# TGAC/KAT

Hardware: AMD Instinct MI355X
Metric: k-mers/sec (whole node) for kat comp reads-vs-assembly k=27 (higher is better)
Workload: dtype u64

## Files before the change

kat_amd/csrc/kg_count.hip:

```cpp
#include "kg_host.hpp"
#include "kg_ingest.hpp"
#include "kg_kernels.hpp"
#include "kg_partition.hpp"
#include "kg_partition_wide.hpp"

#include <condition_variable>
#include <deque>
#include <mutex>
#include <thread>


static const uint64_t g_test_sweep_thr = hook("KATGPU_TEST_SWEEP_THR") ? strtoull(hook("KATGPU_TEST_SWEEP_THR"), nullptr, 10) : 0;
static const uint64_t g_test_max_starts = hook("KATGPU_TEST_MAX_STARTS") ? strtoull(hook("KATGPU_TEST_MAX_STARTS"), nullptr, 10) : 0;

namespace kg {
static __global__ void __launch_bounds__(256)
k_sweep(DevTable t, uint32_t thr, unsigned long long* scratch) {
    uint32_t mx = 0;
    const uint64_t stride = (uint64_t)gridDim.x * blockDim.x;
    for (uint64_t i = (uint64_t)blockIdx.x * blockDim.x + threadIdx.x; i < t.cap; i += stride) {
        uint32_t c = t.counts[i];
        if (c >= thr) {
            uint64_t key = t.keys[i];
            uint32_t take = (c / thr) * thr;
// ... 51 lines not shown
    if ((reinterpret_cast<uintptr_t>(dev_bases) & 15) == 0)
        hipLaunchKernelGGL(k_count<true>, dim3(grid), dim3(COUNT_BLOCK), 0, c->stream, t->dev(), dev_bases, (uint64_t)n, n_chunks);
    else
        hipLaunchKernelGGL(k_count<false>, dim3(grid), dim3(COUNT_BLOCK), 0, c->stream, t->dev(), dev_bases, (uint64_t)n, n_chunks);
    HIPCHK(c, hipGetLastError());
    return KATGPU_OK;
}



static const uint64_t g_part_min_starts = getenv("KATGPU_PART_MIN_STARTS") ? strtoull(getenv("KATGPU_PART_MIN_STARTS"), nullptr, 10) : (32ULL << 20);
static const uint64_t g_test_round_items = hook("KATGPU_TEST_ROUND_ITEMS") ? strtoull(hook("KATGPU_TEST_ROUND_ITEMS"), nullptr, 10) : 0;
static const double g_arena_fraction = getenv("KATGPU_ARENA_FRACTION") ? std::min(0.95, std::max(0.05, atof(getenv("KATGPU_ARENA_FRACTION")))) : 0.85;
static const uint32_t g_p1_wgs = hook("KATGPU_P1_WGS") ? std::max<uint32_t>(1, (uint32_t)strtoul(hook("KATGPU_P1_WGS"), nullptr, 10)) : 3;
static const uint32_t g_l1_fast = hook("KATGPU_L1_FAST") ? (uint32_t)strtoul(hook("KATGPU_L1_FAST"), nullptr, 10) : 1;
static const uint32_t g_test_l1_cpb = hook("KATGPU_TEST_L1_CPB") ? (uint32_t)strtoul(hook("KATGPU_TEST_L1_CPB"), nullptr, 10) : 0;
static const uint32_t g_p2_fast = hook("KATGPU_P2_FAST") ? (uint32_t)strtoul(hook("KATGPU_P2_FAST"), nullptr, 10) : 1;
static const uint64_t g_test_p2_ovf_cap = hook("KATGPU_TEST_P2_OVF_CAP") ? strtoull(hook("KATGPU_TEST_P2_OVF_CAP"), nullptr, 10) : 0;
static const uint32_t g_test_spill_mod = hook("KATGPU_TEST_SPILL_MOD") ? (uint32_t)strtoul(hook("KATGPU_TEST_SPILL_MOD"), nullptr, 10) : 0;
static const uint64_t g_test_ap_seg = hook_u64("KATGPU_TEST_AP_SEG", 0) & ~3ULL;
static const uint32_t g_apply_per_cu = (uint32_t)hook_u64("KATGPU_APPLY_PER_CU", 0);
static const uint64_t g_fresh_max_pct = hook_u64("KATGPU_FRESH_MAX_PCT", 100);
static const bool g_l1b_stamp = hook_u64("KATGPU_L1B_STAMP", 0) != 0;
static const bool g_p2x_stamp = hook_u64("KATGPU_P2X_STAMP", 0) != 0;
static const bool g_p2_stamp = hook_u64("KATGPU_P2_STAMP", 0) != 0;
static const bool g_apply_stamp = hook_u64("KATGPU_APPLY_STAMP", 0) != 0;

static bool part_geometry(const DevTable& d, PartGeom* g) {
    g->R = d.n_regions; g->S = d.region_slots; g->P1 = d.p1; g->P2 = d.p2; g->l2 = d.l2;
    g->b_lo = 0; g->b_hi = d.p1;
// ... 219 lines not shown
    switch (g.hb) {
    case 0: rc = apply_kv12_shape<0>(a, blk, big, fresh, hooked); break;
    case 1: rc = apply_kv12_shape<1>(a, blk, big, fresh, hooked); break;
    case 2: rc = apply_kv12_shape<2>(a, blk, big, fresh, hooked); break;
    case 4: rc = apply_kv12_shape<4>(a, blk, big, fresh, hooked); break;
    }
    if (rc) return rc;
    HIPCHK(c, hipGetLastError());
    return KATGPU_OK;
}

constexpr uint8_t GUARD_BYTE = 0xA5;
struct PartArena {
    uint32_t hb, passes, n_cu; uint64_t regions; bool blocks_shape; double per_item_max; size_t small_bytes;
    uint32_t* hist1; uint64_t* offs; uint64_t* l1_off; uint64_t* off2; uint32_t* cnt2; uint64_t* bend; unsigned long long* spill_n; unsigned long long* ovf_n;
    uint8_t* l1_buf;
    uint8_t* l2_buf;
    uint64_t* ovf_buf; uint64_t ovf_cap;
    ArenaCarve cv;
    size_t round_items, l1_bytes, l2_items;
    PartArena(const PartGeom& g0, uint32_t k, uint32_t W, uint32_t n_cu_) : hb(g0.hb), passes(std::max<uint32_t>(1, g0.P1 / pass_buckets(g0.P1, n_cu_))), n_cu(n_cu_), regions(g0.R), blocks_shape(l1_blocks_shape(g0, k)) {
        per_item_max = arena_bytes_per_item(hb, passes, false, false);
        small_bytes = align_up((size_t)W * MAX_PARTS * 4, 256) + align_up((size_t)W * MAX_PARTS * 8, 256) +
                      align_up((MAX_PARTS + 1) * 8, 256) + align_up(((size_t)MAX_PARTS * MAX_PARTS + 1) * 8, 256) +
                      align_up((size_t)MAX_PARTS * MAX_PARTS * 4, 256) + align_up((size_t)MAX_PARTS * 8, 256) + align_up((size_t)MAX_PARTS * 4, 256) + 256;
    }
    size_t fixed_bytes(uint32_t W) const { return small_bytes + (size_t)arena_fixed_bytes(hb, passes, W, n_cu, false, false); }
    bool carve_from(uint8_t* a, size_t arena_bytes, uint32_t W, size_t want_items) {
        uint8_t* const a0 = a;
        hist1 = carve<uint32_t>(a, (size_t)W * MAX_PARTS * 4);
        offs = carve<uint64_t>(a, (size_t)W * MAX_PARTS * 8);
        l1_off = carve<uint64_t>(a, (MAX_PARTS + 1) * 8);
        off2 = carve<uint64_t>(a, ((size_t)MAX_PARTS * MAX_PARTS + 1) * 8);
        cnt2 = carve<uint32_t>(a, (size_t)MAX_PARTS * MAX_PARTS * 4);
        bend = carve<uint64_t>(a, (size_t)MAX_PARTS * 8);
        carve<uint32_t>(a, (size_t)MAX_PARTS * 4);
        spill_n = carve<unsigned long long>(a, STAMP_AREA * 8);
        ovf_n = spill_n + 1;
        if ((size_t)(a - a0) > small_bytes || arena_bytes <= small_bytes) return false;
        cv = arena_carve(arena_bytes - small_bytes, want_items, hb, passes, W, n_cu, regions, blocks_shape, g_l1_fast, g_test_p2_ovf_cap);
        round_items = cv.round_items; l1_bytes = cv.l1_bytes; l2_items = cv.l2_items; ovf_cap = cv.ovf_cap;
        l1_buf = a;
        l2_buf = l1_buf + cv.l1_bytes + ARENA_GUARD;
        ovf_buf = (uint64_t*)(l2_buf + cv.l2_bytes + ARENA_GUARD);
        return (size_t)((uint8_t*)(ovf_buf + ovf_cap) + ARENA_GUARD - a0) <= arena_bytes;
    }
    uint8_t* guard(int i) const { return i == 0 ? l1_buf + cv.l1_bytes : i == 1 ? l2_buf + cv.l2_bytes : (uint8_t*)(ovf_buf + ovf_cap); }
};
static const char* const GUARD_NAME[3] = {"level-1 buffer", "level-2 buffer", "overflow list"};
static int guards_set(katgpu_ctx* c, const PartArena& A) {
    if (!g_testing) return KATGPU_OK;
    for (int i = 0; i < 3; ++i) HIPCHK(c, hipMemsetAsync(A.guard(i), GUARD_BYTE, ARENA_GUARD, c->stream));
    return KATGPU_OK;
// ... 23 lines not shown
    return t->dv.k == 32 && !t->dv.canonical ? restore_ones(t) : KATGPU_OK;
}

enum class L1Edition { Blocks, SegLean512, SegLean1024, SegPlain512, SegPlain1024, ExactLean, ExactPlain };
static const char* const L1_EDITION_NAME[] = {"Blocks", "SegLean512", "SegLean1024", "SegPlain512", "SegPlain1024", "ExactLean", "ExactPlain"};
struct L1Plan {
    L1Edition edition; bool seg ; uint32_t wgs ; uint64_t n_tiles, tiles_per_wg;
    uint64_t seg_cap, cap_plain, stride64;
};
static L1Plan plan_level1(const PartGeom& g, uint32_t k, size_t m, uint64_t est_items, uint32_t W, uint32_t n_cu, size_t l1_bytes, bool seg_wanted) {
    const bool lean = g_l1_lean && lean_applies(k, g.pl.n1);
    const bool pb512 = g.P1 <= 512;
    const bool l1b = l1_blocks_shape(g, k);
    const uint64_t n_tiles = (m + P1_TILE_STARTS - 1) / P1_TILE_STARTS;
    L1Plan pl;
    pl.wgs = l1b ? n_cu : W;
    pl.n_tiles = l1b ? (m + L1B_TILE_STARTS - 1) / L1B_TILE_STARTS : n_tiles;
    const L1Segments sg = l1_segments(l1b, g.P1, g.hb1, pl.wgs, est_items, (pl.n_tiles + pl.wgs - 1) / pl.wgs, g_test_l1_cpb, l1_bytes);
    pl.cap_plain = sg.cap_plain; pl.seg_cap = sg.seg_cap; pl.stride64 = sg.stride;
    pl.seg = seg_wanted && sg.fits;
    if (pl.seg) pl.edition = l1b ? L1Edition::Blocks : lean ? (pb512 ? L1Edition::SegLean512 : L1Edition::SegLean1024) : (pb512 ? L1Edition::SegPlain512 : L1Edition::SegPlain1024);
    else { pl.edition = lean ? L1Edition::ExactLean : L1Edition::ExactPlain; pl.wgs = W; pl.n_tiles = n_tiles; }
    pl.tiles_per_wg = (pl.n_tiles + pl.wgs - 1) / pl.wgs;
    return pl;
}
static int launch_l1_scatter(katgpu_table* t, const PartGeom& g, const L1Plan& l1, const PartArena& A, const uint8_t* p, uint64_t nb) {
    katgpu_ctx* c = t->ctx;
    auto blocks = [&](auto kern, unsigned long long* stamps) {
        return launch_lds(c, kern, dim3(l1.wgs), dim3(L1B_THREADS), sizeof(P1BLds), sizeof(P1BLds), t->dv, g, p, nb, l1.n_tiles, l1.tiles_per_wg,
                          A.l1_buf, (uint32_t)(l1.seg_cap / L1B_ITEMS), (uint32_t)l1.stride64, A.ovf_buf, A.ovf_n, A.ovf_cap, stamps);
    };
    auto segmented = [&](auto kern) {
        hipLaunchKernelGGL(kern, dim3(l1.wgs), dim3(P1_BLOCK), 0, c->stream, t->dv, g, p, nb, l1.n_tiles, l1.tiles_per_wg, (const uint64_t*)nullptr, (const uint64_t*)nullptr, A.l1_buf,
                           (uint32_t)l1.seg_cap, (uint32_t)l1.stride64, (uint32_t)l1.cap_plain, A.ovf_buf, A.ovf_n, A.ovf_cap);
        return KATGPU_OK;
    };
    auto exact = [&](auto kern) {
        hipLaunchKernelGGL(kern, dim3(l1.wgs), dim3(P1_BLOCK), 0, c->stream, t->dv, g, p, nb, l1.n_tiles, l1.tiles_per_wg, (const uint64_t*)A.offs, (const uint64_t*)A.l1_off, A.l1_buf,
                           0u, 0u, 0u, (uint64_t*)nullptr, (unsigned long long*)nullptr, (uint64_t)0);
        return KATGPU_OK;
    };
    switch (l1.edition) {
    case L1Edition::Blocks:
        if (!g_l1b_stamp) return blocks(k_p1b_scatter<false>, nullptr);
        return with_stamps(c, A.spill_n + STAMP_AT, 10, &STAMPS_L1B, [&](unsigned long long* st) { return blocks(k_p1b_scatter<true>, st); });
    case L1Edition::SegLean512:   return segmented(k_p1v2_scatter<true, true, 512>);
    case L1Edition::SegLean1024:  return segmented(k_p1v2_scatter<true, true, MAX_PARTS>);
    case L1Edition::SegPlain512:  return segmented(k_p1v2_scatter<true, false, 512>);
    case L1Edition::SegPlain1024: return segmented(k_p1v2_scatter<true, false, MAX_PARTS>);
    case L1Edition::ExactLean:    return exact(k_p1v2_scatter<false, true, MAX_PARTS>);
    case L1Edition::ExactPlain:   return exact(k_p1v2_scatter<false, false, MAX_PARTS>);
    }
    return KATGPU_OK;
}
static int level1(katgpu_table* t, const PartGeom& g, const L1Plan& l1, const PartArena& A, size_t cap_items, const uint8_t* p, size_t m, double items_per_start, uint64_t* items) {
    katgpu_ctx* c = t->ctx;
    const uint64_t nb = m + t->dv.k - 1;
    if (l1.seg) {
        int rc;
        if (l1.stride64 * g.P1 > A.l1_bytes || (uint64_t)l1.wgs * (l1.edition == L1Edition::Blocks ? l1.seg_cap / L1B_ITEMS * L1B_BYTES : (4 + g.hb1) * l1.seg_cap) > l1.stride64)
// ... 11 lines not shown
    HIPCHK(c, hipMemcpyAsync(items, &A.l1_off[g.P1], sizeof *items, hipMemcpyDeviceToHost, c->stream));
    HIPCHK(c, hipStreamSynchronize(c->stream));
    if (g_trace) fprintf(stderr, "[katgpu] partition round: %zu starts -> %llu items (buffer %zu items, arena %.1f GB, ratio %.3f; capacity %zu items, %s, stride 0)\n", m, (unsigned long long)*items, A.round_items, c->arena_bytes / 1e9, items_per_start,
                         cap_items, L1_EDITION_NAME[(int)l1.edition]);
    if (*items > cap_items) return t->dv.k == 32 && !t->dv.canonical ? restore_ones(t) : KATGPU_OK;
    if (!*items) return KATGPU_OK;
    if (l1_bucket_base(*items, g.P1) + 32 > A.l1_bytes)
        return fail(c, KATGPU_ERR_DEVICE, "partition round: %llu items of an exact level 1 end beyond the level-1 buffer of %zu bytes", (unsigned long long)*items, A.l1_bytes);
    ScopedTimer tm(c, KATGPU_K_PART_L1S, *items);
    return launch_l1_scatter(t, g, l1, A, p, nb);
}

enum class L1Items { Groups , WideGroups , Blocks  };
static const char* const L1_ITEMS_NAME[] = {"Groups", "WideGroups", "Blocks"};
enum L2Family : uint32_t { L2_BLOCKS = 1 , L2_ONE_PASS = 2 , L2_EXACT = 4  };
struct L2Pass { katgpu_ctx* c; const PartGeom& g; const PartArena& A; uint32_t grid; L1Items src; uint64_t seg_slots; uint32_t* families ; };
template <typename K>
static int p2_one_pass(const L2Pass& x, K kern, size_t lds, unsigned long long* stamps = nullptr) {
    return launch_lds(x.c, kern, dim3(x.grid), dim3(PART_BLOCK), lds, lds, x.g, x.A.l1_off, x.A.l1_buf, x.A.l2_buf, x.A.off2, x.A.cnt2, x.A.ovf_buf, x.A.ovf_n, x.A.ovf_cap, x.seg_slots, stamps);
}
template <typename K>
static int p2_exact(const L2Pass& x, K kern, size_t lds) {
    return launch_lds(x.c, kern, dim3(x.grid), dim3(PART_BLOCK), lds, lds, x.g, x.A.l1_off, x.A.l1_buf, x.A.l2_buf, x.A.off2, x.seg_slots, x.A.bend);
}
template <int HB>
static int launch_l2_hb(const L2Pass& x, bool one_pass) {
    constexpr size_t lds_e = sizeof(P2Lds<HB>), lds_f = sizeof(typename P2FastLds<HB>::type);
    unsigned long long* const stamps = x.A.spill_n + STAMP_AT;
    if (x.families) *x.families |= !one_pass ? L2_EXACT : x.src == L1Items::Blocks && HB == 1 ? L2_BLOCKS : L2_ONE_PASS;
    switch (x.src) {
    case L1Items::Blocks:
        if constexpr (HB == 4) break;
        else if (!one_pass) return p2_exact(x, k_p2<HB, false, true>, lds_e);
        else if constexpr (HB != 1) return p2_one_pass(x, k_p2_fast<HB, false, false, true>, lds_f);
        else if (!g_p2x_stamp) return p2_one_pass(x, k_p2x_fast<false>, sizeof(P2XLds));
        else return with_stamps(x.c, stamps, 10, &STAMPS_P2X, [&](unsigned long long* st) { return p2_one_pass(x, k_p2x_fast<true>, sizeof(P2XLds), st); });
    case L1Items::WideGroups: return one_pass ? p2_one_pass(x, k_p2_fast<HB, true>, lds_f) : p2_exact(x, k_p2<HB, true>, lds_e);
    case L1Items::Groups:
        if constexpr (HB == 1) if (one_pass && g_p2_stamp) return with_stamps(x.c, stamps, 6, &STAMPS_P2, [&](unsigned long long* st) { return p2_one_pass(x, k_p2_fast<1, false, true>, lds_f, st); });
        return one_pass ? p2_one_pass(x, k_p2_fast<HB, false>, lds_f) : p2_exact(x, k_p2<HB, false>, lds_e);
    }
    return fail(x.c, KATGPU_ERR_DEVICE, "level 2 from blocked level-1 items: item width %u", x.g.hb);
}
static int launch_l2(const L2Pass& x, bool one_pass) {
    switch (x.g.hb) {
    case 0: return launch_l2_hb<0>(x, one_pass);
    case 1: return launch_l2_hb<1>(x, one_pass);
    case 2: return launch_l2_hb<2>(x, one_pass);
    case 4: return launch_l2_hb<4>(x, one_pass);
    }
    return fail(x.c, KATGPU_ERR_DEVICE, "level 2: item width %u", x.g.hb);
// ... 39 lines not shown
    };
    uint32_t step = pass_buckets(g.P1, (uint32_t)c->n_cu);
    auto fits = [&](uint32_t st) { for (uint32_t b = 0; b < g.P1; b += st) if (pass_extent(b, std::min(g.P1, b + st)) > A.l2_items) return false; return true; };
    if (!seg && A.cv.big) {
        g.l2_trim = 0;
        if (!fits(step) && l2_trims(g.hb, items, g.R)) g.l2_trim = 1;
    }
    while (step > 1 && !fits(step)) step = (step + 1) / 2;
    if (!fits(step)) {
        *end = RoundEnd::DirectPath;
        return seg || (t->dv.k == 32 && !t->dv.canonical) ? restore_ones(t) : KATGPU_OK;
    }
    const bool try_fast0 = *p2_fast_ok && (g_p2_fast == 2 || items / g.R >= 1024);
    unsigned long long ovf_total = ovf_l1;
    uint32_t l2_families = 0;
    ApplyForm ap{};
    if (g_trace && g.P1 > step) fprintf(stderr, "[katgpu]   level 2 + apply in %u passes of %u buckets (level-2 buffer: %zu items)\n", (g.P1 + step - 1) / step, step, A.l2_items);
    for (uint32_t b_lo = 0; b_lo < g.P1; b_lo += step) {
        g.b_lo = b_lo; g.b_hi = std::min(g.P1, b_lo + step);
        const uint64_t pass_items = std::max<uint64_t>(1, (uint64_t)((double)items * (g.b_hi - g.b_lo) / g.P1));
        auto l1_at = [&](uint32_t b) -> uint64_t { return seg ? (uint64_t)b * g.l1_stride : l1_bucket_base(lbeg(b), b); };
        uint64_t* spill_buf = (uint64_t*)(A.l1_buf + l1_at(b_lo));
        g.spill_cap = (l1_at(g.b_hi) - l1_at(b_lo)) / 8;
        const bool try_fast = try_fast0 && *p2_fast_ok;
        const L2Pass x{c, g, A, std::min<uint32_t>(g.b_hi - g.b_lo, (uint32_t)c->n_cu), src, seg_slots, &l2_families};
        HIPCHK(c, hipMemsetAsync(A.spill_n, 0, sizeof(unsigned long long), c->stream));
        int rc = KATGPU_OK;
        if (try_fast) { ScopedTimer tm(c, KATGPU_K_PART_L2, pass_items); rc = launch_l2(x, true); }
        if (rc) return rc;
        L2Next next = L2Next::Exact;
        unsigned long long overflowed = ovf_total;
        if (try_fast || (seg && b_lo == 0)) {
            rc = read_overflow(t, A, seg, try_fast, ovf_l1, &ovf_total, &overflowed, &next);
            if (rc) return rc;
            if (next == L2Next::RedoRound) { *end = RoundEnd::RedoExactL1; return KATGPU_OK; }
            if (next == L2Next::FallBackExact) *p2_fast_ok = false;
        }
        const bool runs = next == L2Next::UseCnt2;
        if (!runs) { ScopedTimer tm(c, KATGPU_K_PART_L2, pass_items); rc = launch_l2(x, false); }
        if (rc) return rc;
        ovf_total = overflowed;
        {
            ScopedTimer tm(c, KATGPU_K_PART_APPLY, pass_items);
            rc = launch_apply(t, g, A.off2, A.l2_buf, spill_buf, A.spill_n, runs ? A.cnt2 : nullptr, runs ? nullptr : A.bend, items, &ap);
// ... 527 lines not shown
```

kat_amd/csrc/kg_l1_blocks.hpp:

```cpp
#pragma once

namespace kg {

constexpr uint32_t L1B_ITEMS = 10, L1B_BYTES = 64;
constexpr int L1B_THREADS = 1024;
constexpr int L1B_TILE_BYTES = L1B_THREADS * PART_ITEMS;
constexpr int L1B_TILE_STARTS = L1B_TILE_BYTES - CHUNK_OVERLAP;
constexpr int L1B_LANES_WITH_STARTS = L1B_TILE_STARTS / PART_ITEMS;
constexpr uint32_t L1B_PB = 512;
constexpr uint32_t L1B_POOL = 1712;

struct P1BLds {
    uint32_t hist[L1B_PB + 64];
    uint2 gb[L1B_PB + 64];
    uint32_t where[L1B_POOL];
    uint32_t wave_tot[L1B_THREADS / 64];
    uint32_t code[L1B_THREADS + 2];
    uint16_t bad[L1B_THREADS + 2];
    __attribute__((aligned(16))) uint32_t img[(L1B_PB + L1B_POOL) * 16];
};
static_assert(sizeof(P1BLds) <= 160 * 1024 - 1280, "one workgroup per CU");

__device__ __forceinline__ uint32_t l1b_lo_at(uint32_t B, uint32_t s) { return B + 3 * (s >> 1) + (s & 1); }
__device__ __forceinline__ uint32_t l1b_hi_at(uint32_t B, uint32_t s) { return 2 * (B + 3 * (s >> 1) + 2) + (s & 1); }
// ... 8 lines not shown
#pragma unroll
    for (uint32_t i = 0; i < 4; ++i) {
        const uint32_t b = (tid_o & ~63u) + 16 * i + ((tid_o & 63) >> 2);
        const uint2 d = L.gb[b];
        if (d.x & 0xFFFFu) {
            const u32x4 a = *reinterpret_cast<const u32x4*>(&L.img[b * 16 + (tid_o & 3) * 4]);
            *reinterpret_cast<u32x4*>(&L.img[d.y * 16 + (tid_o & 3) * 4]) = a;
        }
    }
}

template <bool STAMP = false >
__global__ void __launch_bounds__(L1B_THREADS)
k_p1b_scatter(DevTable t, PartGeom g, const uint8_t* __restrict__ bases, uint64_t n, uint64_t n_tiles, uint64_t tiles_per_wg,
              uint8_t* __restrict__ l1_buf, uint32_t segb , uint32_t bucket_stride ,
              uint64_t* __restrict__ ovf_buf, unsigned long long* __restrict__ ovf_n, uint64_t ovf_cap, unsigned long long* __restrict__ stamps) {
    constexpr uint32_t PB = L1B_PB;
    unsigned long long st[10] = {0, 0, 0, 0, 0, 0, 0, 0, 0, 0}, tq = 0;
    auto stamp = [&](int i) { if (STAMP) { const unsigned long long x = (unsigned long long)clock64(); st[i] += x - tq; tq = x; } };
    extern __shared__ __attribute__((aligned(16))) unsigned char lds_raw[];
    P1BLds& L = *reinterpret_cast<P1BLds*>(lds_raw);
    const uint32_t tid = threadIdx.x, P = g.P1, k = t.k;
    uint16_t* const img16 = reinterpret_cast<uint16_t*>(L.img);
    uint8_t* const seg0 = l1_buf + (uint64_t)blockIdx.x * segb * L1B_BYTES;
    const LeanGeom lg = lean_geom(k, t.canonical != 0, g.pl.n1);
    auto overflow = [&](uint32_t b, uint32_t lo, uint32_t hi) {
        const unsigned long long at = atomicAdd(ovf_n, 1ULL);
        if (at < ovf_cap) ovf_buf[at] = place_key_r1(b, ((uint64_t)hi << 32) | lo, g.pl);
    };
    if (tid < PB + 64) { L.hist[tid] = 0; L.gb[tid] = uint2{0u, 0u}; }
    if (tid < PB) L.img[tid * 16 + 15] = 0;
// ... 148 lines not shown
        const bool room = cur < segb;
        if (cn && !room) {
            for (uint32_t s = 0; s < cn; ++s) overflow(tid, L.img[l1b_lo_at(tid * 16, s)], img16[l1b_hi_at(tid * 16, s)]);
        }
        if (cn && room) for (uint32_t s = cn; s < L1B_ITEMS; ++s) { L.img[l1b_lo_at(tid * 16, s)] = 0xFFFFFFFFu; img16[l1b_hi_at(tid * 16, s)] = 0xFFFFu; }
        L.gb[tid].x = cn && room ? 1u : 0u;
    }
    lds_barrier();
    for (uint32_t qi = tid; qi < 4 * P; qi += L1B_THREADS) {
        const uint32_t b = qi >> 2, w = qi & 3;
        const uint32_t cur = L.img[b * 16 + 15];
        u32x4 v = *reinterpret_cast<const u32x4*>(&L.img[b * 16 + 4 * w]);
        if (w == 3) v.w = 0xFFFFFFFFu;
        if (L.gb[b].x) *reinterpret_cast<u32x4*>(seg0 + ((uint64_t)b * bucket_stride + ((uint64_t)cur << 6) + 16 * w)) = v;
    }
    lds_barrier();
    {
        const uint32_t wave = tid >> 6, lane = tid & 63;
        for (uint32_t b = wave; b < P; b += L1B_THREADS / 64) {
            const uint32_t from = L.img[b * 16 + 15] + L.gb[b].x;
            uint8_t* seg = seg0 + (uint64_t)b * bucket_stride;
            for (uint32_t q = from * 4 + lane; q < segb * 4; q += 64) *reinterpret_cast<u32x4*>(seg + (uint64_t)q * 16) = u32x4{0xFFFFFFFFu, 0xFFFFFFFFu, 0xFFFFFFFFu, 0xFFFFFFFFu};
        }
    }
}

}
```

kat_amd/csrc/kg_l2_blocks.hpp:

```cpp
#pragma once

namespace kg {

constexpr int L2X_N = 14;
constexpr uint32_t L2X_TILE = L2X_N * PART_BLOCK;
constexpr uint32_t L2X_POOL = 1252;

struct P2XLds {
    uint32_t hist[MAX_PARTS + 64];
    uint2 gb[MAX_PARTS];
    uint32_t where[L2X_POOL];
    uint32_t wave_tot[32];
    __attribute__((aligned(64))) uint32_t img[(MAX_PARTS + L2X_POOL) * 16];
};
static_assert(sizeof(P2XLds) <= 160 * 1024 - 256 && offsetof(P2XLds, img) % 64 == 0, "LDS");
static_assert(PART_BLOCK == MAX_PARTS, "thread b is sub-bucket b");

template <bool STAMP = false >
__global__ void __launch_bounds__(PART_BLOCK)
k_p2x_fast(PartGeom g, const uint64_t* __restrict__ l1_off, const uint8_t* __restrict__ l1_buf, uint8_t* __restrict__ l2_buf,
           uint64_t* __restrict__ off2, uint32_t* __restrict__ cnt2, uint64_t* __restrict__ ovf_buf, unsigned long long* __restrict__ ovf_n,
           uint64_t ovf_cap, uint64_t seg_slots, unsigned long long* __restrict__ stamps) {
    constexpr int N = L2X_N;
    constexpr uint32_t PB = MAX_PARTS, TILE_CAP = L2Fmt<1>::TILE ;
    extern __shared__ __attribute__((aligned(64))) unsigned char lds_raw[];
    P2XLds& L = *reinterpret_cast<P2XLds*>(lds_raw);
    unsigned char* const img8 = reinterpret_cast<unsigned char*>(L.img);
    const uint32_t tid = threadIdx.x, P = g.P2;
    unsigned long long st[10] = {0, 0, 0, 0, 0, 0, 0, 0, 0, 0}, tq = 0;
    auto stamp = [&](int i) { if (STAMP) { const unsigned long long x = (unsigned long long)clock64(); st[i] += x - tq; tq = x; } };
    uint64_t beg0, n0, nr0;
    l1_bucket_range(g, l1_off, seg_slots, g.b_lo, beg0, n0, nr0);
    uint32_t tid_o = tid;
    for (uint32_t b1 = g.b_lo + blockIdx.x; b1 < g.b_hi; b1 += gridDim.x) {
        uint64_t beg, n_items, n_real;
        const uint8_t* bucket = l1_buf + l1_bucket_range(g, l1_off, seg_slots, b1, beg, n_items, n_real);
        const uint64_t cap = p2_region_cap(n_real, P, TILE_CAP, L2_BLOCK_ITEMS, g.l2_trim != 0);
        const uint64_t obase = p2_out_base(beg, b1, P, TILE_CAP, L2_BLOCK_ITEMS, g.l2_trim != 0) - p2_out_base(beg0, g.b_lo, P, TILE_CAP, L2_BLOCK_ITEMS, g.l2_trim != 0);
        uint8_t* const runs = l2_buf + l2_lo_at<1>(obase >> 2);
        const uint32_t capb = (uint32_t)(cap / L2_BLOCK_ITEMS);
        lds_barrier();
        asm volatile("" : "+v"(tid_o));
        L.hist[tid_o] = 0; L.gb[tid_o] = uint2{0u, 0u};
        if (tid < 64) L.hist[PB + tid_o] = 0;
        L.img[tid_o * 16 + 15] = 0;
        if (tid < P) off2[(uint64_t)b1 * P + tid_o] = obase + (uint64_t)tid * cap;
        uint32_t n_out = 0;
        constexpr int OUT_STEPS = (L2X_POOL + PART_BLOCK / 4 - 1) / (PART_BLOCK / 4);
        static_assert(OUT_STEPS <= N / 2, "a step per pair of the ranking's items");
        struct OutStep { u32x4 v; uint32_t where; };
        auto out_read = [&](int it, OutStep& o) {
            asm volatile("" : "+v"(tid_o));
            const uint32_t s = min((tid_o >> 2) + (uint32_t)it * (PART_BLOCK / 4), L2X_POOL - 1);
            o.where = L.where[s];
            o.v = *reinterpret_cast<const u32x4*>(&L.img[(PB + s) * 16 + (tid_o & 3) * 4]);
        };
        auto out_store = [&](int it, const OutStep& o) {
            asm volatile("" : "+v"(tid_o));
            if ((tid_o >> 2) + (uint32_t)it * (PART_BLOCK / 4) < n_out)
                *reinterpret_cast<u32x4*>(runs + (((uint64_t)o.where << 6) | ((tid_o & 3) * 16))) = o.v;
        };
        RawTileB<N> raw;
        p2_tile_issue_l1b<N>(bucket, 0, raw);
        for (uint64_t tbeg = 0; tbeg < n_items; tbeg += L2X_TILE) {
            if (STAMP) tq = (unsigned long long)clock64();
            TileItems<N, false> key;
            const uint32_t valid = p2_tile_decode_l1b<N>(tbeg, n_items, raw, key);
            {
#pragma unroll
                for (int j = 0; j < N; ++j) asm volatile("" : "+v"(key.lo[j]));
#pragma unroll
                for (int j = 0; j < N / 2; ++j) asm volatile("" : "+v"(key.hi[j]));
            }
            p2_tile_issue_l1b<N>(bucket, tbeg + L2X_TILE, raw);
            stamp(0);
            lds_barrier();
            stamp(1);
            uint32_t br[N];
            {
                uint32_t rk[N];
                const uint32_t dump = PB + (tid & 63);
                OutStep o;
#pragma unroll
                for (int j = 0; j < N; ++j) {
                    if (j % 2 == 0 && j / 2 < OUT_STEPS) out_read(j / 2, o);
                    const uint32_t b = place_digit2_of(key.r1(j), g.pl) & (PB - 1);
                    rk[j] = atomicAdd(&L.hist[(valid >> j & 1) ? b : dump], 1u);
                    br[j] = b << 16;
                    if (j >= 2) br[j - 2] |= rk[j - 2];
// ... 114 lines not shown
```

kat_amd/csrc/kg_partition.hpp:

```cpp
#pragma once
#include "kg_kernels.hpp"
#include "kg_l1_lean.hpp"
#include "kg_apply_lean.hpp"
#include "kg_arena_plan.hpp"

#include <cstddef>
#include <type_traits>

namespace kg {

constexpr int PART_BLOCK = 1024;
constexpr int PART_ITEMS = BASES_PER_LANE;
constexpr int TILE_ITEMS = PART_BLOCK * PART_ITEMS;
constexpr int L1_TILE_BYTES = TILE_ITEMS;
constexpr int L1_TILE_STARTS = L1_TILE_BYTES - CHUNK_OVERLAP;
constexpr int L1_LANES_WITH_STARTS = L1_TILE_STARTS / PART_ITEMS;

__device__ __forceinline__ void lds_barrier() { asm volatile("s_waitcnt lgkmcnt(0)\n\ts_barrier" ::: "memory"); }
__device__ __forceinline__ void spill_put(uint64_t* __restrict__ spill, unsigned long long* __restrict__ spill_n, uint64_t cap, uint64_t key) {
    const unsigned long long at = atomicAdd(spill_n, 1ULL);
    if (at < cap) spill[at] = key;
}

struct PartGeom {
// ... 526 lines not shown
        for (int off = 32; off > 0; off >>= 1) ones += __shfl_down(ones, off, 64);
        if ((tid & 63) == 0 && ones) atomicAdd((unsigned long long*)&t.ctrs[CTR_ONES], (unsigned long long)ones);
    }
}

}
#include "kg_l1_blocks.hpp"
namespace kg {

__device__ __forceinline__ uint64_t l1_bucket_range(const PartGeom& g, const uint64_t* __restrict__ l1_off, uint64_t seg_slots, uint32_t b1, uint64_t& first, uint64_t& n_items, uint64_t& n_real) {
    if (seg_slots) { first = (uint64_t)b1 * g.l1_real; n_items = seg_slots; n_real = g.l1_real; return (uint64_t)b1 * g.l1_stride; }
    first = l1_off[b1]; n_items = n_real = l1_off[b1 + 1] - first;
    return l1_bucket_base(first, b1);
}

template <int N, bool W1>
struct TileItems {
    uint32_t lo[N];
    uint32_t hi[W1 ? N : N / 2];
    __device__ __forceinline__ uint64_t r1(int j) const {
        const uint32_t h = W1 ? hi[j] : (hi[j >> 1] >> (16 * (j & 1))) & 0xFFFFu;
        return ((uint64_t)h << 32) | lo[j];
    }
};
template <int N>
__device__ __forceinline__ uint32_t p2_tile_load_wide(const uint8_t* __restrict__ bucket, uint64_t tbeg, uint64_t n_items, TileItems<N, true>& it) {
    static_assert(N % 2 == 0, "pairs");
    const uint64_t left = n_items - tbeg;
    const uint32_t t_items = left < (uint64_t)N * PART_BLOCK ? (uint32_t)left : (uint32_t)N * PART_BLOCK;
    const uint8_t* mine = bucket + (tbeg + 2 * threadIdx.x) * 8;
// ... 55 lines not shown
    p2_tile_issue_narrow<N>(hb1, bucket, tbeg, r);
    return p2_tile_decode_narrow<N>(hb1, tbeg, n_items, r, it);
}
typedef uint32_t u32x3 __attribute__((ext_vector_type(3)));
typedef u32x3 u32x3_a4 __attribute__((aligned(4)));
template <int N> struct RawTileB { u32x3 v[N / 2]; };
template <int N>
__device__ __forceinline__ void p2_tile_issue_l1b(const uint8_t* __restrict__ bucket, uint64_t tbeg, RawTileB<N>& r) {
    const uint32_t p0 = (uint32_t)(tbeg >> 1) + threadIdx.x;
    uint32_t blk = __umulhi(p0, 0xCCCCCCCDu) >> 2, part = p0 - 5 * blk;
#pragma unroll
    for (int u = 0; u < N / 2; ++u) {
        r.v[u] = *reinterpret_cast<const u32x3_a4*>(bucket + (uint32_t)((blk << 6) + 12 * part));
        blk += PART_BLOCK / 5; part += PART_BLOCK % 5;
        if (part >= 5) { part -= 5; ++blk; }
    }
}
template <int N>
__device__ __forceinline__ uint32_t p2_tile_decode_l1b(uint64_t tbeg, uint64_t n_items, const RawTileB<N>& r, TileItems<N, false>& it) {
    const uint64_t left = tbeg < n_items ? n_items - tbeg : 0;
    const uint32_t t_items = left < (uint64_t)N * PART_BLOCK ? (uint32_t)left : (uint32_t)N * PART_BLOCK;
    uint32_t valid = 0;
#pragma unroll
    for (int u = 0; u < N / 2; ++u) {
        const uint32_t i0 = 2 * ((uint32_t)u * PART_BLOCK + threadIdx.x);
        it.lo[2 * u] = r.v[u].x; it.lo[2 * u + 1] = r.v[u].y; it.hi[u] = r.v[u].z;
        uint32_t ta = (i0 < t_items && !(r.v[u].x == 0xFFFFFFFFu && (r.v[u].z & 0xFFFFu) == 0xFFFFu)) ? 1u : 0u;
        uint32_t tb = (i0 + 1 < t_items && !(r.v[u].y == 0xFFFFFFFFu && (r.v[u].z >> 16) == 0xFFFFu)) ? 1u : 0u;
        asm volatile("" : "+v"(ta), "+v"(tb));
        valid |= (ta << (2 * u)) | (tb << (2 * u + 1));
// ... 1091 lines not shown
```

Measured before the change: 114.9 billion.

## Read only filled level-1 segments via per-bucket fill prefix sums

The level-1 blocks scatter no longer pads every unused segment tail with 0xFF sentinels. It records each workgroup's filled block count per bucket, and a small scan kernel turns these into per-bucket prefix sums. The one-pass level-2 reader for hb==1 uses the prefix sums to map logical blocks onto physical segment positions, so it only walks filled blocks. Other level-2 paths still get a lazy padding kernel. This removes padding writes and reads of empty capacity, at the cost of an extra scan launch and more address arithmetic in the L2 tile loads.

```diff
diff --git a/kat_amd/csrc/kg_count.hip b/kat_amd/csrc/kg_count.hip
--- a/kat_amd/csrc/kg_count.hip
+++ b/kat_amd/csrc/kg_count.hip
@@ -89,6 +89,7 @@
 static const double g_arena_fraction = getenv("KATGPU_ARENA_FRACTION") ? std::min(0.95, std::max(0.05, atof(getenv("KATGPU_ARENA_FRACTION")))) : 0.85;
 static const uint32_t g_p1_wgs = hook("KATGPU_P1_WGS") ? std::max<uint32_t>(1, (uint32_t)strtoul(hook("KATGPU_P1_WGS"), nullptr, 10)) : 3;
 static const uint32_t g_l1_fast = hook("KATGPU_L1_FAST") ? (uint32_t)strtoul(hook("KATGPU_L1_FAST"), nullptr, 10) : 1;
+static const uint32_t g_test_l1b_wgs = (uint32_t)hook_u64("KATGPU_TEST_L1B_WGS", 0);
 static const uint32_t g_test_l1_cpb = hook("KATGPU_TEST_L1_CPB") ? (uint32_t)strtoul(hook("KATGPU_TEST_L1_CPB"), nullptr, 10) : 0;
 static const uint32_t g_p2_fast = hook("KATGPU_P2_FAST") ? (uint32_t)strtoul(hook("KATGPU_P2_FAST"), nullptr, 10) : 1;
 static const uint64_t g_test_p2_ovf_cap = hook("KATGPU_TEST_P2_OVF_CAP") ? strtoull(hook("KATGPU_TEST_P2_OVF_CAP"), nullptr, 10) : 0;
@@ -338,6 +339,7 @@
 struct PartArena {
     uint32_t hb, passes, n_cu; uint64_t regions; bool blocks_shape; double per_item_max; size_t small_bytes;
     uint32_t* hist1; uint64_t* offs; uint64_t* l1_off; uint64_t* off2; uint32_t* cnt2; uint64_t* bend; unsigned long long* spill_n; unsigned long long* ovf_n;
+    uint32_t* l1_fill; uint32_t* l1_cum;
     uint8_t* l1_buf;
     uint8_t* l2_buf;
     uint64_t* ovf_buf; uint64_t ovf_cap;
@@ -347,8 +349,11 @@
         per_item_max = arena_bytes_per_item(hb, passes, false, false);
         small_bytes = align_up((size_t)W * MAX_PARTS * 4, 256) + align_up((size_t)W * MAX_PARTS * 8, 256) +
                       align_up((MAX_PARTS + 1) * 8, 256) + align_up(((size_t)MAX_PARTS * MAX_PARTS + 1) * 8, 256) +
-                      align_up((size_t)MAX_PARTS * MAX_PARTS * 4, 256) + align_up((size_t)MAX_PARTS * 8, 256) + align_up((size_t)MAX_PARTS * 4, 256) + 256;
-    }
+                      align_up((size_t)MAX_PARTS * MAX_PARTS * 4, 256) + align_up((size_t)MAX_PARTS * 8, 256) + align_up((size_t)MAX_PARTS * 4, 256) + 256 +
+                      align_up(fill_bytes(), 256) + align_up(cum_bytes(), 256);
+    }
+    size_t fill_bytes() const { return (size_t)n_cu * L1B_PB * 4; }
+    size_t cum_bytes() const { return ((size_t)n_cu + 1) * L1B_PB * 4; }
     size_t fixed_bytes(uint32_t W) const { return small_bytes + (size_t)arena_fixed_bytes(hb, passes, W, n_cu, false, false); }
     bool carve_from(uint8_t* a, size_t arena_bytes, uint32_t W, size_t want_items) {
         uint8_t* const a0 = a;
@@ -361,6 +366,8 @@
         carve<uint32_t>(a, (size_t)MAX_PARTS * 4);
         spill_n = carve<unsigned long long>(a, STAMP_AREA * 8);
         ovf_n = spill_n + 1;
+        l1_fill = carve<uint32_t>(a, fill_bytes());
+        l1_cum = carve<uint32_t>(a, cum_bytes());
         if ((size_t)(a - a0) > small_bytes || arena_bytes <= small_bytes) return false;
         cv = arena_carve(arena_bytes - small_bytes, want_items, hb, passes, W, n_cu, regions, blocks_shape, g_l1_fast, g_test_p2_ovf_cap);
         round_items = cv.round_items; l1_bytes = cv.l1_bytes; l2_items = cv.l2_items; ovf_cap = cv.ovf_cap;
@@ -414,7 +421,7 @@
     const bool l1b = l1_blocks_shape(g, k);
     const uint64_t n_tiles = (m + P1_TILE_STARTS - 1) / P1_TILE_STARTS;
     L1Plan pl;
-    pl.wgs = l1b ? n_cu : W;
+    pl.wgs = l1b ? (g_test_l1b_wgs ? std::min(g_test_l1b_wgs, n_cu) : n_cu) : W;
     pl.n_tiles = l1b ? (m + L1B_TILE_STARTS - 1) / L1B_TILE_STARTS : n_tiles;
     const L1Segments sg = l1_segments(l1b, g.P1, g.hb1, pl.wgs, est_items, (pl.n_tiles + pl.wgs - 1) / pl.wgs, g_test_l1_cpb, l1_bytes);
     pl.cap_plain = sg.cap_plain; pl.seg_cap = sg.seg_cap; pl.stride64 = sg.stride;
@@ -428,7 +435,7 @@
     katgpu_ctx* c = t->ctx;
     auto blocks = [&](auto kern, unsigned long long* stamps) {
         return launch_lds(c, kern, dim3(l1.wgs), dim3(L1B_THREADS), sizeof(P1BLds), sizeof(P1BLds), t->dv, g, p, nb, l1.n_tiles, l1.tiles_per_wg,
-                          A.l1_buf, (uint32_t)(l1.seg_cap / L1B_ITEMS), (uint32_t)l1.stride64, A.ovf_buf, A.ovf_n, A.ovf_cap, stamps);
+                          A.l1_buf, (uint32_t)(l1.seg_cap / L1B_ITEMS), (uint32_t)l1.stride64, A.ovf_buf, A.ovf_n, A.ovf_cap, A.l1_fill, stamps);
     };
     auto segmented = [&](auto kern) {
         hipLaunchKernelGGL(kern, dim3(l1.wgs), dim3(P1_BLOCK), 0, c->stream, t->dv, g, p, nb, l1.n_tiles, l1.tiles_per_wg, (const uint64_t*)nullptr, (const uint64_t*)nullptr, A.l1_buf,
@@ -441,9 +448,14 @@
         return KATGPU_OK;
     };
     switch (l1.edition) {
-    case L1Edition::Blocks:
-        if (!g_l1b_stamp) return blocks(k_p1b_scatter<false>, nullptr);
-        return with_stamps(c, A.spill_n + STAMP_AT, 10, &STAMPS_L1B, [&](unsigned long long* st) { return blocks(k_p1b_scatter<true>, st); });
+    case L1Edition::Blocks: {
+        if (g_testing) HIPCHK(c, hipMemsetAsync(A.l1_buf, 0x01, l1.stride64 * g.P1, c->stream));
+        int rc = !g_l1b_stamp ? blocks(k_p1b_scatter<false>, nullptr)
+                              : with_stamps(c, A.spill_n + STAMP_AT, 10, &STAMPS_L1B, [&](unsigned long long* st) { return blocks(k_p1b_scatter<true>, st); });
+        if (rc) return rc;
+        hipLaunchKernelGGL(k_l1_fill_scan, dim3(g.P1), dim3(64), 0, c->stream, (const uint32_t*)A.l1_fill, A.l1_cum, l1.wgs);
+        return KATGPU_OK;
+    }
     case L1Edition::SegLean512:   return segmented(k_p1v2_scatter<true, true, 512>);
     case L1Edition::SegLean1024:  return segmented(k_p1v2_scatter<true, true, MAX_PARTS>);
     case L1Edition::SegPlain512:  return segmented(k_p1v2_scatter<true, false, 512>);
@@ -485,10 +497,27 @@
 enum class L1Items { Groups , WideGroups , Blocks  };
 static const char* const L1_ITEMS_NAME[] = {"Groups", "WideGroups", "Blocks"};
 enum L2Family : uint32_t { L2_BLOCKS = 1 , L2_ONE_PASS = 2 , L2_EXACT = 4  };
-struct L2Pass { katgpu_ctx* c; const PartGeom& g; const PartArena& A; uint32_t grid; L1Items src; uint64_t seg_slots; uint32_t* families ; };
+struct L2Pass {
+    katgpu_ctx* c; const PartGeom& g; const PartArena& A; uint32_t grid; L1Items src; uint64_t seg_slots; uint32_t* families ;
+    uint32_t wgs, segb;
+    bool* padded;
+};
 template <typename K>
 static int p2_one_pass(const L2Pass& x, K kern, size_t lds, unsigned long long* stamps = nullptr) {
     return launch_lds(x.c, kern, dim3(x.grid), dim3(PART_BLOCK), lds, lds, x.g, x.A.l1_off, x.A.l1_buf, x.A.l2_buf, x.A.off2, x.A.cnt2, x.A.ovf_buf, x.A.ovf_n, x.A.ovf_cap, x.seg_slots, stamps);
+}
+template <typename K>
+static int p2_blocks(const L2Pass& x, K kern, unsigned long long* stamps = nullptr) {
+    const size_t lds = sizeof(P2XLds);
+    return launch_lds(x.c, kern, dim3(x.grid), dim3(PART_BLOCK), lds, lds, x.g, x.A.l1_off, x.A.l1_buf, x.A.l2_buf, x.A.off2, x.A.cnt2, x.A.ovf_buf, x.A.ovf_n, x.A.ovf_cap, x.seg_slots,
+                      (const uint32_t*)x.A.l1_cum, x.wgs, x.segb, stamps);
+}
+static int pad_blocks(const L2Pass& x) {
+    if (*x.padded) return KATGPU_OK;
+    hipLaunchKernelGGL(k_l1_pad_segments, dim3((x.g.P1 - x.g.b_lo) * x.wgs), dim3(256), 0, x.c->stream, (const uint32_t*)x.A.l1_fill, x.A.l1_buf, x.wgs, x.segb, x.g.l1_stride, x.g.b_lo);
+    *x.padded = true;
+    if (g_trace) fprintf(stderr, "[katgpu]   level-1 segments of buckets %u .. %u filled up with \"no item\" (k_l1_pad_segments): the reader takes whole segments\n", x.g.b_lo, x.g.P1 - 1);
+    return KATGPU_OK;
 }
 template <typename K>
 static int p2_exact(const L2Pass& x, K kern, size_t lds) {
@@ -502,10 +531,10 @@
     switch (x.src) {
     case L1Items::Blocks:
         if constexpr (HB == 4) break;
-        else if (!one_pass) return p2_exact(x, k_p2<HB, false, true>, lds_e);
-        else if constexpr (HB != 1) return p2_one_pass(x, k_p2_fast<HB, false, false, true>, lds_f);
-        else if (!g_p2x_stamp) return p2_one_pass(x, k_p2x_fast<false>, sizeof(P2XLds));
-        else return with_stamps(x.c, stamps, 10, &STAMPS_P2X, [&](unsigned long long* st) { return p2_one_pass(x, k_p2x_fast<true>, sizeof(P2XLds), st); });
+        else if (!one_pass) { int rc = pad_blocks(x); return rc ? rc : p2_exact(x, k_p2<HB, false, true>, lds_e); }
+        else if constexpr (HB != 1) { int rc = pad_blocks(x); return rc ? rc : p2_one_pass(x, k_p2_fast<HB, false, false, true>, lds_f); }
+        else if (!g_p2x_stamp) return p2_blocks(x, k_p2x_fast<false>);
+        else return with_stamps(x.c, stamps, 10, &STAMPS_P2X, [&](unsigned long long* st) { return p2_blocks(x, k_p2x_fast<true>, st); });
     case L1Items::WideGroups: return one_pass ? p2_one_pass(x, k_p2_fast<HB, true>, lds_f) : p2_exact(x, k_p2<HB, true>, lds_e);
     case L1Items::Groups:
         if constexpr (HB == 1) if (one_pass && g_p2_stamp) return with_stamps(x.c, stamps, 6, &STAMPS_P2, [&](unsigned long long* st) { return p2_one_pass(x, k_p2_fast<1, false, true>, lds_f, st); });
@@ -575,6 +604,14 @@
     const bool try_fast0 = *p2_fast_ok && (g_p2_fast == 2 || items / g.R >= 1024);
     unsigned long long ovf_total = ovf_l1;
     uint32_t l2_families = 0;
+    bool padded = false;
+    const uint32_t segb = src == L1Items::Blocks ? (uint32_t)(l1.seg_cap / L1B_ITEMS) : 0u;
+    std::vector<uint32_t> h_cum;
+    if (g_trace && src == L1Items::Blocks) {
+        h_cum.resize((size_t)g.P1 * (l1.wgs + 1));
+        HIPCHK(c, hipMemcpyAsync(h_cum.data(), A.l1_cum, h_cum.size() * 4, hipMemcpyDeviceToHost, c->stream));
+        HIPCHK(c, hipStreamSynchronize(c->stream));
+    }
     ApplyForm ap{};
     if (g_trace && g.P1 > step) fprintf(stderr, "[katgpu]   level 2 + apply in %u passes of %u buckets (level-2 buffer: %zu items)\n", (g.P1 + step - 1) / step, step, A.l2_items);
     for (uint32_t b_lo = 0; b_lo < g.P1; b_lo += step) {
@@ -584,11 +621,17 @@
         uint64_t* spill_buf = (uint64_t*)(A.l1_buf + l1_at(b_lo));
         g.spill_cap = (l1_at(g.b_hi) - l1_at(b_lo)) / 8;
         const bool try_fast = try_fast0 && *p2_fast_ok;
-        const L2Pass x{c, g, A, std::min<uint32_t>(g.b_hi - g.b_lo, (uint32_t)c->n_cu), src, seg_slots, &l2_families};
+        const L2Pass x{c, g, A, std::min<uint32_t>(g.b_hi - g.b_lo, (uint32_t)c->n_cu), src, seg_slots, &l2_families, l1.wgs, segb, &padded};
         HIPCHK(c, hipMemsetAsync(A.spill_n, 0, sizeof(unsigned long long), c->stream));
         int rc = KATGPU_OK;
         if (try_fast) { ScopedTimer tm(c, KATGPU_K_PART_L2, pass_items); rc = launch_l2(x, true); }
         if (rc) return rc;
+        if (try_fast && !h_cum.empty() && g.hb == 1) {
+            unsigned long long read = 0;
+            for (uint32_t b = g.b_lo; b < g.b_hi; ++b) read += h_cum[(size_t)b * (l1.wgs + 1) + l1.wgs];
+            fprintf(stderr, "[katgpu]   level 2 walked buckets %u .. %u compacted: %llu blocks read of %llu blocks of capacity (%u segments of %u per bucket)\n", g.b_lo, g.b_hi - 1, read,
+                    (unsigned long long)(g.b_hi - g.b_lo) * l1.wgs * segb, l1.wgs, segb);
+        }
         L2Next next = L2Next::Exact;
         unsigned long long overflowed = ovf_total;
         if (try_fast || (seg && b_lo == 0)) {
diff --git a/kat_amd/csrc/kg_l1_blocks.hpp b/kat_amd/csrc/kg_l1_blocks.hpp
--- a/kat_amd/csrc/kg_l1_blocks.hpp
+++ b/kat_amd/csrc/kg_l1_blocks.hpp
@@ -46,7 +46,8 @@
 __global__ void __launch_bounds__(L1B_THREADS)
 k_p1b_scatter(DevTable t, PartGeom g, const uint8_t* __restrict__ bases, uint64_t n, uint64_t n_tiles, uint64_t tiles_per_wg,
               uint8_t* __restrict__ l1_buf, uint32_t segb , uint32_t bucket_stride ,
-              uint64_t* __restrict__ ovf_buf, unsigned long long* __restrict__ ovf_n, uint64_t ovf_cap, unsigned long long* __restrict__ stamps) {
+              uint64_t* __restrict__ ovf_buf, unsigned long long* __restrict__ ovf_n, uint64_t ovf_cap, uint32_t* __restrict__ fill ,
+              unsigned long long* __restrict__ stamps) {
     constexpr uint32_t PB = L1B_PB;
     unsigned long long st[10] = {0, 0, 0, 0, 0, 0, 0, 0, 0, 0}, tq = 0;
     auto stamp = [&](int i) { if (STAMP) { const unsigned long long x = (unsigned long long)clock64(); st[i] += x - tq; tq = x; } };
@@ -225,15 +226,7 @@
         if (w == 3) v.w = 0xFFFFFFFFu;
         if (L.gb[b].x) *reinterpret_cast<u32x4*>(seg0 + ((uint64_t)b * bucket_stride + ((uint64_t)cur << 6) + 16 * w)) = v;
     }
-    lds_barrier();
-    {
-        const uint32_t wave = tid >> 6, lane = tid & 63;
-        for (uint32_t b = wave; b < P; b += L1B_THREADS / 64) {
-            const uint32_t from = L.img[b * 16 + 15] + L.gb[b].x;
-            uint8_t* seg = seg0 + (uint64_t)b * bucket_stride;
-            for (uint32_t q = from * 4 + lane; q < segb * 4; q += 64) *reinterpret_cast<u32x4*>(seg + (uint64_t)q * 16) = u32x4{0xFFFFFFFFu, 0xFFFFFFFFu, 0xFFFFFFFFu, 0xFFFFFFFFu};
-        }
-    }
+    if (tid < P) fill[tid * gridDim.x + blockIdx.x] = L.img[tid * 16 + 15] + L.gb[tid].x;
 }
 
 }
diff --git a/kat_amd/csrc/kg_l1_fill.hpp b/kat_amd/csrc/kg_l1_fill.hpp
--- /dev/null
+++ b/kat_amd/csrc/kg_l1_fill.hpp
@@ -0,0 +1,61 @@
+#pragma once
+#include <stdint.h>
+
+#if defined(__HIPCC__)
+#define KG_FILL_FN __host__ __device__ __forceinline__
+#else
+#define KG_FILL_FN inline
+#endif
+
+namespace kg {
+
+constexpr uint32_t FILL_NO_END = 0xFFFFFFFFu;
+
+KG_FILL_FN uint32_t fill_cum_at(const uint32_t* cum, uint32_t wgs, uint32_t i) { return i <= wgs ? cum[i] : FILL_NO_END; }
+KG_FILL_FN uint32_t fill_seg_of(const uint32_t* cum, uint32_t wgs, uint32_t lb, uint32_t lo) {
+    uint32_t hi = wgs + 1;
+    while (hi - lo > 1) {
+        const uint32_t mid = lo + ((hi - lo) >> 1);
+        if (cum[mid] <= lb) lo = mid; else hi = mid;
+    }
+    return lo;
+}
+
+struct FillWalk {
+    uint32_t s0;
+    uint32_t end0;
+    uint32_t end1;
+    uint32_t sh0, sh1;
+};
+KG_FILL_FN FillWalk fill_walk_seek(const uint32_t* cum, uint32_t wgs, uint32_t segb, uint32_t first, uint32_t lo = 0) {
+    FillWalk w;
+    w.s0 = fill_seg_of(cum, wgs, first, lo);
+    w.end0 = fill_cum_at(cum, wgs, w.s0 + 1);
+    w.end1 = fill_cum_at(cum, wgs, w.s0 + 2);
+    w.sh0 = w.s0 * segb - cum[w.s0];
+    w.sh1 = (w.s0 + 1) * segb - w.end0;
+    return w;
+}
+KG_FILL_FN bool fill_walk_holds(const FillWalk& w, uint32_t first) { return first < w.end0; }
+KG_FILL_FN bool fill_two_suffice(const FillWalk& w, uint32_t last) { return last < w.end1; }
+KG_FILL_FN uint32_t fill_phys_two(const FillWalk& w, uint32_t lb) { return lb + (lb < w.end0 ? w.sh0 : w.sh1); }
+KG_FILL_FN uint32_t fill_phys_exact(const uint32_t* cum, uint32_t wgs, uint32_t segb, uint32_t s0, uint32_t lb) {
+    const uint32_t s = fill_seg_of(cum, wgs, lb, s0);
+    return lb + s * segb - cum[s];
+}
+template <int M>
+KG_FILL_FN void fill_shifts_many(const uint32_t* cum, uint32_t wgs, uint32_t segb, const FillWalk& w, uint32_t last, const uint32_t (&blk)[M], uint32_t (&sh)[M]) {
+    for (int u = 0; u < M; ++u) sh[u] = w.sh0;
+    for (uint32_t s = w.s0 + 1; s <= wgs; ++s) {
+        const uint32_t c = cum[s];
+        if (c > last) break;
+        const uint32_t shs = s * segb - c;
+        for (int u = 0; u < M; ++u) sh[u] = blk[u] >= c ? shs : sh[u];
+    }
+}
+
+constexpr uint32_t FILL_PAIRS_PER_BLOCK = 5;
+KG_FILL_FN uint32_t fill_tile_first(uint32_t pair0) { return pair0 / FILL_PAIRS_PER_BLOCK; }
+KG_FILL_FN uint32_t fill_tile_last(uint32_t pair0, uint32_t pairs) { return (pair0 + pairs - 1) / FILL_PAIRS_PER_BLOCK; }
+
+}
diff --git a/kat_amd/csrc/kg_l2_blocks.hpp b/kat_amd/csrc/kg_l2_blocks.hpp
--- a/kat_amd/csrc/kg_l2_blocks.hpp
+++ b/kat_amd/csrc/kg_l2_blocks.hpp
@@ -20,7 +20,8 @@
 __global__ void __launch_bounds__(PART_BLOCK)
 k_p2x_fast(PartGeom g, const uint64_t* __restrict__ l1_off, const uint8_t* __restrict__ l1_buf, uint8_t* __restrict__ l2_buf,
            uint64_t* __restrict__ off2, uint32_t* __restrict__ cnt2, uint64_t* __restrict__ ovf_buf, unsigned long long* __restrict__ ovf_n,
-           uint64_t ovf_cap, uint64_t seg_slots, unsigned long long* __restrict__ stamps) {
+           uint64_t ovf_cap, uint64_t seg_slots, const uint32_t* __restrict__ l1_cum , uint32_t l1_wgs, uint32_t segb,
+           unsigned long long* __restrict__ stamps) {
     constexpr int N = L2X_N;
     constexpr uint32_t PB = MAX_PARTS, TILE_CAP = L2Fmt<1>::TILE ;
     extern __shared__ __attribute__((aligned(64))) unsigned char lds_raw[];
@@ -33,8 +34,19 @@
     l1_bucket_range(g, l1_off, seg_slots, g.b_lo, beg0, n0, nr0);
     uint32_t tid_o = tid;
     for (uint32_t b1 = g.b_lo + blockIdx.x; b1 < g.b_hi; b1 += gridDim.x) {
-        uint64_t beg, n_items, n_real;
-        const uint8_t* bucket = l1_buf + l1_bucket_range(g, l1_off, seg_slots, b1, beg, n_items, n_real);
+        uint64_t beg, n_slots, n_real;
+        const uint8_t* bucket = l1_buf + l1_bucket_range(g, l1_off, seg_slots, b1, beg, n_slots, n_real);
+        const uint32_t* const cum = l1_cum + (uint64_t)b1 * (l1_wgs + 1);
+        const uint64_t n_items = (uint64_t)L1B_ITEMS * (uint32_t)__builtin_amdgcn_readfirstlane((int)cum[l1_wgs]);
+        FillWalk fw = fill_walk_seek(cum, l1_wgs, segb, 0);
+        auto issue = [&](uint64_t tbeg, RawTileB<N>& r) {
+            const uint32_t pair0 = (uint32_t)(tbeg >> 1);
+            const uint32_t first = fill_tile_first(pair0), last = fill_tile_last(pair0, L2X_TILE / 2);
+            if (!fill_walk_holds(fw, first)) fw = fill_walk_seek(cum, l1_wgs, segb, first, fw.s0);
+            fw.s0 = (uint32_t)__builtin_amdgcn_readfirstlane((int)fw.s0); fw.end0 = (uint32_t)__builtin_amdgcn_readfirstlane((int)fw.end0); fw.end1 = (uint32_t)__builtin_amdgcn_readfirstlane((int)fw.end1);
+            fw.sh0 = (uint32_t)__builtin_amdgcn_readfirstlane((int)fw.sh0); fw.sh1 = (uint32_t)__builtin_amdgcn_readfirstlane((int)fw.sh1);
+            p2_tile_issue_l1b_fill<N>(bucket, pair0, fw, last, cum, l1_wgs, segb, r);
+        };
         const uint64_t cap = p2_region_cap(n_real, P, TILE_CAP, L2_BLOCK_ITEMS, g.l2_trim != 0);
         const uint64_t obase = p2_out_base(beg, b1, P, TILE_CAP, L2_BLOCK_ITEMS, g.l2_trim != 0) - p2_out_base(beg0, g.b_lo, P, TILE_CAP, L2_BLOCK_ITEMS, g.l2_trim != 0);
         uint8_t* const runs = l2_buf + l2_lo_at<1>(obase >> 2);
@@ -61,7 +73,7 @@
                 *reinterpret_cast<u32x4*>(runs + (((uint64_t)o.where << 6) | ((tid_o & 3) * 16))) = o.v;
         };
         RawTileB<N> raw;
-        p2_tile_issue_l1b<N>(bucket, 0, raw);
+        issue(0, raw);
         for (uint64_t tbeg = 0; tbeg < n_items; tbeg += L2X_TILE) {
             if (STAMP) tq = (unsigned long long)clock64();
             TileItems<N, false> key;
@@ -72,7 +84,7 @@
 #pragma unroll
                 for (int j = 0; j < N / 2; ++j) asm volatile("" : "+v"(key.hi[j]));
             }
-            p2_tile_issue_l1b<N>(bucket, tbeg + L2X_TILE, raw);
+            issue(tbeg + L2X_TILE, raw);
             stamp(0);
             lds_barrier();
             stamp(1);
diff --git a/kat_amd/csrc/kg_partition.hpp b/kat_amd/csrc/kg_partition.hpp
--- a/kat_amd/csrc/kg_partition.hpp
+++ b/kat_amd/csrc/kg_partition.hpp
@@ -3,6 +3,7 @@
 #include "kg_l1_lean.hpp"
 #include "kg_apply_lean.hpp"
 #include "kg_arena_plan.hpp"
+#include "kg_l1_fill.hpp"
 
 #include <cstddef>
 #include <type_traits>
@@ -564,6 +565,25 @@
     return l1_bucket_base(first, b1);
 }
 
+__global__ void __launch_bounds__(64) k_l1_fill_scan(const uint32_t* __restrict__ fill, uint32_t* __restrict__ cum, uint32_t wgs) {
+    const uint32_t b = blockIdx.x, lane = threadIdx.x;
+    const uint32_t* f = fill + (uint64_t)b * wgs;
+    uint32_t* c = cum + (uint64_t)b * (wgs + 1);
+    uint32_t carry = 0;
+    if (lane == 0) c[0] = 0;
+    for (uint32_t base = 0; base < wgs; base += 64) {
+        const uint32_t inc = wave_inclusive_scan(base + lane < wgs ? f[base + lane] : 0u);
+        if (base + lane < wgs) c[base + lane + 1] = carry + inc;
+        carry += lane_value(inc, 63);
+    }
+}
+__global__ void __launch_bounds__(256) k_l1_pad_segments(const uint32_t* __restrict__ fill, uint8_t* __restrict__ l1_buf, uint32_t wgs, uint32_t segb, uint64_t bucket_stride, uint32_t b_lo) {
+    const uint32_t b = b_lo + blockIdx.x / wgs, w = blockIdx.x % wgs;
+    const uint32_t from = min(fill[(uint64_t)b * wgs + w], segb);
+    uint8_t* seg = l1_buf + (uint64_t)b * bucket_stride + (uint64_t)w * segb * L1B_BYTES;
+    for (uint64_t q = (uint64_t)from * 4 + threadIdx.x; q < (uint64_t)segb * 4; q += 256) *reinterpret_cast<u32x4*>(seg + q * 16) = u32x4{0xFFFFFFFFu, 0xFFFFFFFFu, 0xFFFFFFFFu, 0xFFFFFFFFu};
+}
+
 template <int N, bool W1>
 struct TileItems {
     uint32_t lo[N];
@@ -649,6 +669,27 @@
         r.v[u] = *reinterpret_cast<const u32x3_a4*>(bucket + (uint32_t)((blk << 6) + 12 * part));
         blk += PART_BLOCK / 5; part += PART_BLOCK % 5;
         if (part >= 5) { part -= 5; ++blk; }
+    }
+}
+template <int N>
+__device__ __forceinline__ void p2_tile_issue_l1b_fill(const uint8_t* __restrict__ bucket, uint32_t pair0, const FillWalk& w, uint32_t last, const uint32_t* __restrict__ cum, uint32_t wgs, uint32_t segb,
+                                                       RawTileB<N>& r) {
+    const uint32_t p0 = pair0 + threadIdx.x;
+    uint32_t blk = __umulhi(p0, 0xCCCCCCCDu) >> 2, part = p0 - 5 * blk;
+    if (fill_two_suffice(w, last)) {
+#pragma unroll
+        for (int u = 0; u < N / 2; ++u) {
+            r.v[u] = *reinterpret_cast<const u32x3_a4*>(bucket + (uint32_t)((fill_phys_two(w, blk) << 6) + 12 * part));
+            blk += PART_BLOCK / 5; part += PART_BLOCK % 5;
+            if (part >= 5) { part -= 5; ++blk; }
+        }
+    } else {
+        uint32_t b[N / 2], sh[N / 2];
+#pragma unroll
+        for (int u = 0; u < N / 2; ++u) { b[u] = blk + (uint32_t)u * (PART_BLOCK / 5) + (part + (uint32_t)u * (PART_BLOCK % 5)) / 5; }
+        fill_shifts_many<N / 2>(cum, wgs, segb, w, last, b, sh);
+#pragma unroll
+        for (int u = 0; u < N / 2; ++u) r.v[u] = *reinterpret_cast<const u32x3_a4*>(bucket + (uint32_t)(((b[u] + sh[u]) << 6) + 12 * ((part + (uint32_t)u * (PART_BLOCK % 5)) % 5)));
     }
 }
 template <int N>
```

After: 115.7 billion, median of 6. No clear change (+0.7%).
